# 1Jamie/HMSE

Hardware: AMD Instinct MI355X
Metric: ingest_GiB_per_s (higher is better)
Workload: dtype u8; 1 GPU; full ingest (FastCDC 2/8/32 KiB + SHA-256 dedupe + MinHash-128/LSH 4x32 + dictionary DEFLATE level-9 profile) over 10.00 GB wikipedia; total_bytes=9999220736, seg_size=4194304, collective=none

## Files before the change

### hmse_amd/csrc/l1_deflate.hip

```cpp
#include "common.h"
#include <stdio.h>
#include <stdlib.h>
#include <mutex>

namespace dfl {

constexpr int HB = 12;
constexpr int NBK = 1 << HB;
constexpr uint32_t MINM = 4, MAXM = 258, WMAX = 32768;

__device__ __forceinline__ uint32_t hash4(uint32_t x) { return (x * 0x9E3779B1u) >> (32 - HB); }
__device__ __forceinline__ uint32_t ld32(const uint8_t* p) { uint32_t v; __builtin_memcpy(&v, p, 4); return v; }

__device__ __forceinline__ uint32_t alignb(uint32_t hi, uint32_t lo, uint32_t sh) { return __builtin_amdgcn_alignbyte(hi, lo, sh); }
__device__ __forceinline__ uint32_t ld32a(const uint8_t* W, uint32_t off) {
  const uint32_t* w = (const uint32_t*)(W + (off & ~3u));
  return alignb(w[1], w[0], off);
}
__device__ __forceinline__ void ld64a(const uint8_t* W, uint32_t off, uint32_t& x0, uint32_t& x1) {
  const uint32_t* w = (const uint32_t*)(W + (off & ~3u));
  const uint32_t a = w[0], b = w[1], c = w[2];
  x0 = alignb(b, a, off); x1 = alignb(c, b, off);
}
__device__ __forceinline__ uint32_t sort_key(const uint8_t* W, uint32_t off) {
  const uint32_t* w = (const uint32_t*)(W + (off & ~3u));
  const uint32_t a = w[0], b = w[1];
  return ((alignb(b, a, off) * 0x9E3779B1u) & 0xFFFF0000u) | ((b >> ((off & 3u) * 8u)) & 0x0Fu);
}
template <int N>
__device__ __forceinline__ void ldNa(const uint8_t* W, uint32_t off, uint64_t (&x)[N]) {
  const uint32_t* w = (const uint32_t*)(W + (off & ~3u));
  uint32_t d[2 * N + 1];
#pragma unroll
  for (int u = 0; u < 2 * N + 1; u++) d[u] = w[u];
#pragma unroll
  for (int u = 0; u < N; u++) x[u] = ((uint64_t)alignb(d[2 * u + 2], d[2 * u + 1], off) << 32) | alignb(d[2 * u + 1], d[2 * u], off);
}

__device__ __forceinline__ uint32_t cur_get(const uint32_t* c, uint32_t h) { return (c[h >> 1] >> ((h & 1u) * 16u)) & 0xFFFFu; }
__device__ __forceinline__ uint32_t cur_inc(uint32_t* c, uint32_t h) {
  const uint32_t sh = (h & 1u) * 16u;
  return (atomicAdd(&c[h >> 1], 1u << sh) >> sh) & 0xFFFFu;
}

__device__ __forceinline__ void len_sym(uint32_t len, uint32_t& code, uint32_t& eb, uint32_t& ev) {
  if (len == 258) { code = 285; eb = 0; ev = 0; return; }
  const uint32_t l = len - 3;
  if (l < 8) { code = 257 + l; eb = 0; ev = 0; return; }
  const uint32_t e = (31 - __builtin_clz(l)) - 2;
  code = 257 + 4 * e + 4 + ((l >> e) & 3); eb = e; ev = l & ((1u << e) - 1);
}
__device__ __forceinline__ void dist_sym(uint32_t dist, uint32_t& code, uint32_t& eb, uint32_t& ev) {
  const uint32_t d = dist - 1;
  if (d < 4) { code = d; eb = 0; ev = 0; return; }
  const uint32_t hb = 31 - __builtin_clz(d), e = hb - 1;
  code = 2 * hb + ((d >> e) & 1); eb = e; ev = d & ((1u << e) - 1);
}
__device__ __forceinline__ uint32_t len_extra_bits(uint32_t code) {
  if (code < 265 || code == 285) return 0;
  return (code - 261) >> 2;
}
__device__ __forceinline__ uint32_t dist_extra_bits(uint32_t code) { return code < 4 ? 0 : (code >> 1) - 1; }
__device__ __forceinline__ uint32_t fixed_len(uint32_t s) { return s < 144 ? 8 : s < 256 ? 9 : s < 280 ? 7 : 8; }

__device__ __forceinline__ uint32_t uni32(uint32_t v) { return (uint32_t)__builtin_amdgcn_readfirstlane((int)v); }
__device__ __forceinline__ uint64_t uni64(uint64_t v) { return ((uint64_t)uni32((uint32_t)(v >> 32)) << 32) | uni32((uint32_t)v); }

__device__ __forceinline__ void wave_sync() {
  __builtin_amdgcn_fence(__ATOMIC_ACQ_REL, "wavefront");
  __builtin_amdgcn_wave_barrier();
}

template <int N>
struct HuffScratchT {
  uint32_t key[N];
  uint32_t sorted[N];
  uint32_t w[2 * N];
  uint16_t parent[2 * N];
  uint32_t cnt[32];
};
using HuffL = HuffScratchT<288>;
using HuffD = HuffScratchT<32>;

template <int NT, bool WQ>
struct Small {
  uint32_t lf[288], df[32];
  uint32_t red[NT / 64 + 1];
  uint32_t qhead;
  uint32_t ocnt[4];
  struct { uint32_t ji, job, L, Dl; uint64_t c, cstart, rec_at, dstart; } nx;
  uint32_t pexit[NT / 64], pexit2[NT / 64], pconv[NT / 64];
  uint8_t wtab[WQ ? NT : 64];
};

constexpr int align16(int v) { return (v + 15) & ~15; }

#ifndef HMSE_TCAP_S
#define HMSE_TCAP_S 10048
#define HMSE_TCAP_S2 13952
#define HMSE_TCAP_SG 17408
#define HMSE_TCAP_SG2 22976
#endif
constexpr int NT_S = 1024, TCAP_S = HMSE_TCAP_S, TCAP_S2 = HMSE_TCAP_S2, TCAP_SG = HMSE_TCAP_SG, TCAP_SG2 = HMSE_TCAP_SG2;
constexpr int NT_M = 1024, TCAP_SG3 = 32768;
#ifndef HMSE_NT_B
#define HMSE_NT_B 1024
#endif
constexpr int NT_B = HMSE_NT_B, TCAP_B = 65536, LCAP_B = 32768;

template <int NT, int TCAP, int LCAP_, bool LDSM, bool MDG = false, bool MLG = false, bool NOK = false>
struct Layout {
  static constexpr int LCAP = LCAP_;
  static constexpr int W_OFF = 0;
  static constexpr int W_SZ = align16(TCAP + 64);
  static constexpr int CUR_OFF = W_OFF + W_SZ;
  static constexpr int CUR_SZ = NBK * 2;
  static constexpr int MARK_OFF = CUR_OFF + CUR_SZ;
  static constexpr int MARK_SZ = align16(LCAP / 8 + 16);
  static constexpr int SMALL_OFF = MARK_OFF + MARK_SZ;
  static constexpr int SMALL_SZ = align16((int)sizeof(Small<NT, !LDSM>));
  static constexpr int A_OFF = SMALL_OFF + SMALL_SZ;
  static constexpr int A_SZ = LDSM ? align16(2 * TCAP + 80) : align16(LCAP + 80);
  static constexpr int MD_OFF = A_OFF + A_SZ;
  static constexpr int MD_SZ = (LDSM && !MDG) ? align16(2 * LCAP) : 0;
  static constexpr int ML_OFF = MD_OFF + MD_SZ;
  static constexpr int ML_SZ = (LDSM && !MLG) ? align16(LCAP) : 0;
  static constexpr int K_OFF = ML_OFF + ML_SZ;
  static constexpr int K_SZ = (LDSM && !NOK) ? align16(TCAP + 16) : 0;
  static constexpr int TOTAL = K_OFF + K_SZ;
  static_assert(TOTAL <= 160 * 1024, "one workgroup's LDS image must fit the CU's 160 KiB");
  static_assert(!(LDSM && TCAP <= TCAP_SG2) || TOTAL <= 80 * 1024, "classes S .. SG2 run two workgroups per CU");
  static_assert(sizeof(HuffL) + sizeof(HuffD) <= CUR_SZ, "Huffman scratch must fit the cursor table");
};

template <typename HS>
__device__ void huff_lengths_wave(const uint32_t* freq, uint32_t n, uint32_t limit, uint8_t* lens, HS* hs) {
  const uint32_t lane = lane_id();
  uint32_t used = 0;
  for (uint32_t b = 0; b < n; b += 64) {
    const uint32_t s = b + lane;
    used += (uint32_t)__builtin_popcountll(__ballot(s < n && freq[s] != 0));
  }
  uint32_t dummy0 = 0xFFFFFFFFu, dummy1 = 0xFFFFFFFFu;
  if (used == 0) { dummy0 = 0; dummy1 = 1; }
  else if (used == 1) dummy0 = freq[0] != 0 ? 1u : 0u;
  uint32_t m = 0;
  for (uint32_t b = 0; b < n; b += 64) {
    const uint32_t s = b + lane;
    uint32_t f = s < n ? freq[s] : 0u;
    if (s == dummy0 || s == dummy1) f = 1;
    if (s < n) lens[s] = 0;
    const bool u = f != 0;
    const uint64_t mask = __ballot(u);
    if (u) hs->key[m + (uint32_t)__builtin_popcountll(mask & lanemask_lt())] = (f << 9) | s;
    m += (uint32_t)__builtin_popcountll(mask);
  }
  wave_sync();
  for (uint32_t j = lane; j < m; j += 64) {
    const uint32_t kj = hs->key[j];
    uint32_t r = 0;
    for (uint32_t i = 0; i < m; i++) r += hs->key[i] < kj;
    hs->sorted[r] = kj;
// ... 286 lines not shown
        if (t < a0 - Dl) W[Dl + t] = csrc[t];
        if (t < T - a1) W[a1 + t] = csrc[a1 - Dl + t];
      } else if (t < L) W[Dl + t] = csrc[t];
    }
    if (t < 64) W[T + t] = 0;
    for (uint32_t i = t; i < NBK / 2; i += NT) cur[i] = 0;
    for (uint32_t i = t; i < 288; i += NT) sm.lf[i] = 0;
    if (t < 32) sm.df[t] = 0;
    if (t == 0) sm.qhead = 0;
    if (t < 4) sm.ocnt[t] = 0;
    for (uint32_t i = t * 16; i < L; i += NT * 16) *(uint4*)(mlen + i) = make_uint4(0, 0, 0, 0);
    __syncthreads();

    STAMP(0);
    PF_STAGE(0);
    const uint32_t nh = T >= 4 ? T - 3 : 0;
    for (uint32_t q4 = t * 4u; q4 < nh; q4 += NT * 4u) {
      const uint32_t d0 = *(const uint32_t*)(W + q4), d1 = *(const uint32_t*)(W + q4 + 4u);
      cur_inc(cur, hash4(d0));
      if (q4 + 1u < nh) cur_inc(cur, hash4(alignb(d1, d0, 1u)));
      if (q4 + 2u < nh) cur_inc(cur, hash4(alignb(d1, d0, 2u)));
      if (q4 + 3u < nh) cur_inc(cur, hash4(alignb(d1, d0, 3u)));
    }
    __syncthreads();
    {
      constexpr int PERW = NBK / 2 / NT > 0 ? NBK / 2 / NT : 1;
      uint32_t wv[PERW], sum = 0;
#pragma unroll
      for (int i = 0; i < PERW; i++) {
        const uint32_t idx = t * PERW + i;
        wv[i] = idx < NBK / 2 ? cur[idx] : 0u;
        sum += (wv[i] & 0xFFFFu) + (wv[i] >> 16);
      }
      uint32_t total;
      uint32_t ex = block_exclusive_scan<NT>(sum, sm.red, &total);
#pragma unroll
      for (int i = 0; i < PERW; i++) {
        const uint32_t idx = t * PERW + i;
        const uint32_t lo16 = ex; ex += wv[i] & 0xFFFFu;
        const uint32_t hi16 = ex; ex += wv[i] >> 16;
        if (idx < NBK / 2) cur[idx] = lo16 | (hi16 << 16);
      }
    }
    __syncthreads();
    STAMP(1);
    PF_STAGE(1);
    {
      uint32_t q = t, h = 0, before = 0, hx = 0;
      bool act = q < nh;
      if (act) { hx = sort_key(W, q); h = hx >> (32 - HB); before = cur_get(cur, h); }
      __syncthreads();
      for (uint32_t q0 = 0; q0 < nh; q0 += NT) {
        if (act) S[cur_inc(cur, h)] = (uint16_t)q;
        __syncthreads();
        uint32_t r = 0;
        if (act) {
          const uint32_t after = cur_get(cur, h);
          for (uint32_t jj = before; jj < after; jj++) r += S[jj] < q;
        }
        const uint32_t qn = q0 + NT + t;
        const bool actn = qn < nh;
        uint32_t hn = 0, beforen = 0, hxn = 0;
        if (actn) { hxn = sort_key(W, qn); hn = hxn >> (32 - HB); beforen = cur_get(cur, hn); }
        __syncthreads();
        if (act) { S[before + r] = (uint16_t)q; if constexpr (!NOK) K[before + r] = (uint8_t)((hx & 0x0Fu) | ((hx >> 12) & 0xF0u)); }
        q = qn; act = actn; h = hn; before = beforen; hx = hxn;
      }
      __syncthreads();
    }
    STAMP(2);
    PF_STAGE(2);
    uint32_t* const anch = mark;
    if constexpr (DICT) {
      const uint32_t n_anch = (L + 63u) >> 6;
      for (uint32_t a0 = wave; a0 < n_anch; a0 += NT / 64) {
        const uint32_t pa = Dl + (a0 << 6);
        uint32_t word = 0;
        if (pa + 4 <= T) {
          const uint32_t h = hash4(ld32a(W, pa));
          const uint32_t lo = h ? cur_get(cur, h - 1) : 0u, hi = cur_get(cur, h);
          uint32_t l = lo, r = hi;
          while (l < r) { const uint32_t m = (l + r) >> 1; if ((uint32_t)S[m] < Dl) l = m + 1; else r = m; }
          const uint32_t first = l > lo + 64u ? l - 64u : lo;
          const uint32_t idx = first + lane;
          uint32_t ml = 0, q = 0;
          if (idx < l) {
            q = S[idx];
            if (TCAP <= (int)WMAX || pa - q <= WMAX) {
              uint64_t qa[4], pb[4];
              ldNa<4>(W, q, qa); ldNa<4>(W, pa, pb);
              ml = 32;
#pragma unroll
              for (int u = 3; u >= 0; u--) { const uint64_t x = qa[u] ^ pb[u]; if (x) ml = 8u * u + ((uint32_t)__builtin_ctzll(x) >> 3); }
            }
          }
          uint32_t key = (ml << 8) | lane;
          key = wave_max(key);
          if ((key >> 8) >= 32u) {
            const uint32_t d = pa - (uint32_t)__builtin_amdgcn_readlane((int)q, (int)(key & 63u));
            const uint32_t off = 8u * lane;
            uint32_t n = 8;
            if (pa + off < T) {
              uint64_t xa[1], xb[1];
              ldNa<1>(W, pa + off - d, xa); ldNa<1>(W, pa + off, xb);
              const uint64_t x = xa[0] ^ xb[0];
              if (x) n = (uint32_t)__builtin_ctzll(x) >> 3;
            } else n = 0;
            const uint64_t mm = __ballot(n < 8u);
            uint32_t run = 512;
            if (mm) { const uint32_t fl = (uint32_t)__builtin_ctzll(mm); run = 8u * fl + (uint32_t)__builtin_amdgcn_readlane((int)n, (int)fl); }
            if (run > T - pa) run = T - pa;
            word = d | (run << 16);
          }
        }
        anch[a0] = word;
      }
      __syncthreads();
    }
    auto hint_of = [&](uint32_t p, uint32_t maxlen, uint32_t& bq) -> uint32_t {
      const uint32_t a0 = (p - Dl) >> 6;
      uint32_t bm = 0; bq = 0;
#pragma unroll
      for (uint32_t back = 0; back < 2; back++) {
        if (a0 < back) continue;
        const uint32_t w = anch[a0 - back];
        const uint32_t d = w & 0xFFFFu, run = w >> 16, pa = Dl + ((a0 - back) << 6);
        if (w == 0 || p < pa || d > p || p - d >= Dl) continue;
        uint32_t m = 0;
        if (run >= 512u) m = maxlen;
        else if (pa + run > p) m = (pa + run - p) < maxlen ? (pa + run - p) : maxlen;
        if (m > bm) { bm = m; bq = p - d; }
      }
      return bm;
    };
    if constexpr (DICT) {
      for (uint32_t x = t; x < L; x += NT) {
        const uint32_t p = Dl + x;
        if (p + 4 > T) continue;
        const uint32_t maxlen = (T - p) < MAXM ? (T - p) : MAXM;
        uint32_t bq;
        const uint32_t bm = hint_of(p, maxlen, bq);
        if (bm >= 16u) { mlen[x] = (uint8_t)(bm - 3); mdist[x] = (uint16_t)(p - bq); }
      }
    }
#if defined(HMSE_NO_ORD)
    constexpr bool ORD = false;
#elif defined(HMSE_NO_DICT_ORD)
    constexpr bool ORD = !DICT && LDSM;
#else
    constexpr bool ORD = LDSM;
#endif
    uint32_t* const ord = (uint32_t*)(a.scratch2 + (size_t)blockIdx.x * a.scratch2_stride + 98304u);
    if constexpr (ORD) {
      constexpr int ITER = (TCAP + NT - 1) / NT;
      const uint32_t wv = uni32(wave);
      uint32_t pk[(ITER + 2) / 3];
#pragma unroll
      for (int w = 0; w < (ITER + 2) / 3; w++) pk[w] = 0;
      uint32_t n0 = 0, n1 = 0, n2 = 0, n3 = 0;
      {
        const uint32_t last = nh ? nh - 1u : 0u;
        constexpr int G = DICT ? 2 : ITER > 12 ? 4 : 8;
#pragma unroll
        for (int g = 0; g < ITER; g += G) {
          uint32_t pv[G], hv[G], lv[G];
#pragma unroll
          for (int u = 0; u < G; u++) if (g + u < ITER) { const uint32_t r = (wv << 6) + (uint32_t)(g + u) * NT + lane; pv[u] = S[r < last ? r : last]; }
#pragma unroll
          for (int u = 0; u < G; u++) if (g + u < ITER) hv[u] = ld32a(W, pv[u]) * 0x9E3779B1u;
#pragma unroll
          for (int u = 0; u < G; u++) if (g + u < ITER) lv[u] = cur_get(cur, ((hv[u] >> (32 - HB)) - 1u) & (uint32_t)(NBK - 1));
#pragma unroll
          for (int u = 0; u < G; u++) if (g + u < ITER) {
            const int it = g + u;
            const uint32_t r = (wv << 6) + (uint32_t)it * NT + lane;
            uint32_t km = r - ((hv[u] >> (32 - HB)) ? lv[u] : 0u);
            km = km < a.depth ? km : a.depth;
            km = km < 63u ? km : 63u;
            km = r < nh ? km : 0u;
            if constexpr (DICT) {
              const uint32_t pp = pv[u];
              uint32_t bq;
              const uint32_t bm = pp >= Dl ? hint_of(pp, (T - pp) < MAXM ? (T - pp) : MAXM, bq) : 16u;
              km = bm >= 16u ? 0u : km;
            }
            pk[it / 3] |= (km | ((hv[u] >> 10) & 0x3C0u)) << (10 * (it % 3));
            n0 += (uint32_t)__builtin_popcountll(__ballot(km >= 24u)); n1 += (uint32_t)__builtin_popcountll(__ballot(km >= 12u && km < 24u));
            n2 += (uint32_t)__builtin_popcountll(__ballot(km >= 4u && km < 12u)); n3 += (uint32_t)__builtin_popcountll(__ballot(km >= 1u && km < 4u));
          }
        }
      }
      uint32_t bv = 0;
      if (lane < 4u) bv = atomicAdd(&sm.ocnt[lane], lane == 0u ? n0 : lane == 1u ? n1 : lane == 2u ? n2 : n3);
      uint32_t b0 = (uint32_t)__builtin_amdgcn_readlane((int)bv, 0), b1 = (uint32_t)__builtin_amdgcn_readlane((int)bv, 1),
               b2 = (uint32_t)__builtin_amdgcn_readlane((int)bv, 2), b3 = (uint32_t)__builtin_amdgcn_readlane((int)bv, 3);
      __syncthreads();
      {
        const uint32_t c0 = uni32(sm.ocnt[0]), c1 = uni32(sm.ocnt[1]), c2 = uni32(sm.ocnt[2]);
        b1 += c0; b2 += c0 + c1; b3 += c0 + c1 + c2;
      }
#pragma unroll
      for (int it = 0; it < ITER; it++) {
        const uint32_t r0 = (wv << 6) + (uint32_t)it * NT;
        if (r0 < nh) {
          const uint32_t kv = (pk[it / 3] >> (10 * (it % 3))) & 0x3FFu, km = kv & 63u;
          const uint64_t m0 = __ballot(km >= 24u), m1 = __ballot(km >= 12u && km < 24u), m2 = __ballot(km >= 4u && km < 12u), m3 = __ballot(km >= 1u && km < 4u);
          if (km != 0u) {
            const uint64_t mm = km >= 24u ? m0 : km >= 12u ? m1 : km >= 4u ? m2 : m3;
            const uint32_t pos = (km >= 24u ? b0 : km >= 12u ? b1 : km >= 4u ? b2 : b3) + mbcnt64(mm);
            ord[pos] = (r0 + lane) | (kv << 15);
          }
          b0 += (uint32_t)__builtin_popcountll(m0); b1 += (uint32_t)__builtin_popcountll(m1);
          b2 += (uint32_t)__builtin_popcountll(m2); b3 += (uint32_t)__builtin_popcountll(m3);
        }
      }
      __syncthreads();
      STAMP(8);
    }
    STAMP(6);
    PF_STAGE(3);
    {
      enum { FETCH = 0, PROBE = 1, EXTEND = 2, DONE = 3 };
#ifndef HMSE_FETCH_BATCH
#define HMSE_FETCH_BATCH 16
#endif
#ifndef HMSE_FETCH_BATCH_DICT
#define HMSE_FETCH_BATCH_DICT 8
#endif
      constexpr uint32_t FETCH_BATCH = DICT ? HMSE_FETCH_BATCH_DICT : HMSE_FETCH_BATCH;
      uint32_t st = FETCH, i = 0, p = 0, kk = 0, kmax = 0, best = 0, bd = 0, probe = 0, maxlen = 0, ml = 0, q = 0, qn = 0, kn = 0;
      uint32_t pw0 = 0, pw1 = 0;
#ifndef HMSE_NO_PROBE16
      uint32_t pw2 = 0, pw3 = 0;
#endif
      uint32_t pkey = 0;
      auto rejects = [&](uint32_t kb) -> bool {
        if constexpr (NOK) return best >= 4 && kb != (pw1 & 0xFFu);
        else { const uint32_t x = kb ^ pkey; return (x & 0xF0u) != 0 || (best >= 4 && (x & 0x0Fu) != 0); }
      };
      uint64_t wq_mask = 0; uint32_t wq_base = 0; bool wq_done = false;
      const uint32_t nh_s = uni32(nh);
      const uint32_t n_ord = ORD ? uni32(sm.ocnt[0]) + uni32(sm.ocnt[1]) + uni32(sm.ocnt[2]) + uni32(sm.ocnt[3]) : nh_s;
      uint8_t* const wtab = sm.wtab + (wave << 6);
      auto begin_walk = [&](uint32_t ii, uint32_t pp) {
        i = ii; p = pp;
        qn = i ? S[i - 1] : 0u;
        kn = NOK ? (uint32_t)W[qn + 4] : (i ? (uint32_t)K[i - 1] : 0u);
#ifndef HMSE_NO_PROBE16
        { uint64_t pp__[2]; ldNa<2>(W, p, pp__); pw0 = (uint32_t)pp__[0]; pw1 = (uint32_t)(pp__[0] >> 32); pw2 = (uint32_t)pp__[1]; pw3 = (uint32_t)(pp__[1] >> 32); }
#else
        ld64a(W, p, pw0, pw1);
#endif
        const uint32_t hxp = pw0 * 0x9E3779B1u;
        const uint32_t h = hxp >> (32 - HB);
        pkey = (pw1 & 0x0Fu) | ((hxp >> 12) & 0xF0u);
        const uint32_t lo = h ? cur_get(cur, h - 1) : 0u;
        maxlen = (T - p) < MAXM ? (T - p) : MAXM;
        kmax = i - lo;
        if (kmax > a.depth) kmax = a.depth;
        best = MINM - 1; bd = 0; probe = pw0; kk = 1;
#ifdef HMSE_DFL_STAMPS
        if (DICT && t == 0) stamp_acc[7]++;
#endif
        if (kmax != 0) st = PROBE;
      };
      auto begin_walk_listed = [&](uint32_t e) {
        i = e & 0x7FFFu; kmax = (e >> 15) & 63u;
        p = S[i];
        qn = S[i - 1];
        kn = NOK ? (uint32_t)W[qn + 4] : (uint32_t)K[i - 1];
#ifndef HMSE_NO_PROBE16
        { uint64_t pp__[2]; ldNa<2>(W, p, pp__); pw0 = (uint32_t)pp__[0]; pw1 = (uint32_t)(pp__[0] >> 32); pw2 = (uint32_t)pp__[1]; pw3 = (uint32_t)(pp__[1] >> 32); }
#else
        ld64a(W, p, pw0, pw1);
#endif
        pkey = (pw1 & 0x0Fu) | ((e >> 17) & 0xF0u);
        if (kmax == 63u) {
          const uint32_t h = hash4(pw0), lo = h ? cur_get(cur, h - 1) : 0u;
          kmax = i - lo < a.depth ? i - lo : a.depth;
        }
        maxlen = (T - p) < MAXM ? (T - p) : MAXM;
        best = MINM - 1; bd = 0; probe = pw0; kk = 1;
#ifdef HMSE_DFL_STAMPS
        if (DICT && t == 0) stamp_acc[7]++;
#endif
        st = PROBE;
      };
      const uint32_t trip_budget = (nh + 64u) * (a.depth + 16u);
      uint32_t trips = 0;
      for (;;) {
#ifdef HMSE_DFL_STAMPS
        if (t == 0) stamp_acc[13]++;
#endif
        if (++trips > uni32(trip_budget)) {
#ifdef HMSE_DIAG
          const uint64_t sf = __ballot(st == FETCH), sp = __ballot(st == PROBE), se = __ballot(st == EXTEND);
          if (lane == 0) printf("[dfl] trip budget: job %u k %llu L %u Dl %u nh %u wave %u qhead %u wq_base %u wq_mask %llx wq_done %d FETCH %llx PROBE %llx EXTEND %llx p %u kk %u kmax %u best %u ml %u maxlen %u q %u\n",
                                ji, (unsigned long long)k, L, Dl, nh, wave, sm.qhead, wq_base, (unsigned long long)wq_mask, (int)wq_done, (unsigned long long)sf, (unsigned long long)sp, (unsigned long long)se, p, kk, kmax, best, ml, maxlen, q);
#endif
          if (lane == 0) atomicOr(a.status, 16u);
          break;
        }
        uint64_t need = uni64(__ballot(st == FETCH));
        if constexpr (DICT && !ORD) {
          for (int it = 0; need != 0 && it < 6; it++) {
            if (wq_mask == 0) {
              if (wq_done) break;
              uint32_t b = 0;
              if (lane == 0) b = atomicAdd(&sm.qhead, 64u);
              b = uni32(b);
              if (b >= nh_s) { wq_done = true; break; }
              wq_base = b;
              const uint32_t ii = b + lane;
              bool work = false;
              if (ii < nh_s) {
                const uint32_t pp = S[ii];
                if (pp >= Dl) {
                  const uint32_t mx = (T - pp) < MAXM ? (T - pp) : MAXM;
                  uint32_t bq;
                  const uint32_t bm = hint_of(pp, mx, bq);
                  work = bm < 16u;
                }
              }
              wq_mask = uni64(__ballot(work));
              if (wq_mask == 0) continue;
            }
            const uint32_t navail = (uint32_t)__builtin_popcountll(wq_mask), nneed = (uint32_t)__builtin_popcountll(need);
            const uint32_t take_n = navail < nneed ? navail : nneed;
            const bool has = (wq_mask >> lane) & 1ull;
            const uint32_t rm = mbcnt64(wq_mask);
            if (has && rm < take_n) wtab[rm] = (uint8_t)lane;
            wave_sync();
            const bool isneed = (need >> lane) & 1ull;
            const uint32_t rn = mbcnt64(need);
            uint32_t got = 0xFFFFFFFFu;
            if (isneed && rn < take_n) got = wq_base + (uint32_t)wtab[rn];
            wave_sync();
            wq_mask &= ~uni64(__ballot(has && rm < take_n));
            need &= ~uni64(__ballot(isneed && rn < take_n));
            if (got != 0xFFFFFFFFu) begin_walk(got, (uint32_t)S[got]);
          }
          if (wq_done && wq_mask == 0 && st == FETCH) st = DONE;
        } else if (need && ((uint32_t)__builtin_popcountll(need) >= FETCH_BATCH || uni64(__ballot(st == PROBE || st == EXTEND)) == 0)) {
          const uint32_t leader = (uint32_t)__builtin_ctzll(need);
          uint32_t base = 0;
          if (lane == leader) base = atomicAdd(&sm.qhead, (uint32_t)__builtin_popcountll(need));
          base = (uint32_t)__builtin_amdgcn_readlane((int)base, (int)leader);
          if (st == FETCH) {
            const uint32_t f = base + mbcnt64(need);
            if (f >= n_ord) st = DONE;
            else if constexpr (ORD) begin_walk_listed(ord[f]);
            else begin_walk(f, (uint32_t)S[f]);
          }
        }
        if (uni64(__ballot(st != DONE)) == 0) break;
#ifdef HMSE_DFL_STAMPS
        const uint64_t occP__ = __ballot(st == PROBE), occE__ = __ballot(st == EXTEND);
        if (t == 0) {
          const uint32_t nP = (uint32_t)__builtin_popcountll(occP__), nE = (uint32_t)__builtin_popcountll(occE__);
          const uint32_t nF = (uint32_t)__builtin_popcountll(need);
          stamp_acc[16] += nF != 0; stamp_acc[17] += nF; stamp_acc[18] += nP != 0; stamp_acc[19] += nP; stamp_acc[20] += nE != 0; stamp_acc[21] += nE;
        }
#endif
        bool fin = false;
#ifdef HMSE_EXT_MIN
        const uint64_t em__ = uni64(__ballot(st == EXTEND));
        const bool run_ext = (uint32_t)__builtin_popcountll(em__) >= (uint32_t)HMSE_EXT_MIN || uni64(__ballot(st == PROBE)) == 0;
#else
        constexpr bool run_ext = true;
#endif
        if (st == PROBE) {
          q = qn;
          uint32_t kb = kn;
          if (kk < kmax) { qn = S[i - kk - 1]; kn = NOK ? (uint32_t)W[qn + 4] : (uint32_t)K[i - kk - 1]; }
          if (!NOK && rejects(kb) && kk < kmax && !(TCAP > (int)WMAX && p - q > WMAX) ) {
            kk++;
            q = qn; kb = kn;
            if (kk < kmax) { qn = S[i - kk - 1]; kn = NOK ? (uint32_t)W[qn + 4] : (uint32_t)K[i - kk - 1]; }
          }
          fin = true; ml = 0;
          if (TCAP > (int)WMAX && p - q > WMAX) kk = kmax;
          else if (rejects(kb)) { }
          else {
            const uint32_t cprobe = ld32a(W, q + best - 3);
            uint32_t c0, c1;
            ld64a(W, q, c0, c1);
            uint32_t x;
            if (cprobe != probe) { }
            else if ((x = c0 ^ pw0) != 0) ml = (uint32_t)__builtin_ctz(x) >> 3;
            else if ((x = c1 ^ pw1) != 0) ml = 4 + ((uint32_t)__builtin_ctz(x) >> 3);
#ifndef HMSE_NO_PROBE16
            else if (maxlen > 8) {
              uint32_t c2, c3;
              ld64a(W, q + 8, c2, c3);
              if ((x = c2 ^ pw2) != 0) ml = 8 + ((uint32_t)__builtin_ctz(x) >> 3);
              else if ((x = c3 ^ pw3) != 0) ml = 12 + ((uint32_t)__builtin_ctz(x) >> 3);
              else { ml = 16; if (maxlen > 16) { fin = false; st = EXTEND; } }
            } else ml = 8;
#else
            else { ml = 8; if (maxlen > 8) { fin = false; st = EXTEND; } }
#endif
          }
        } else if (st == EXTEND && run_ext) {
          if constexpr (!LDSM || TCAP > TCAP_SG2) {
            uint64_t da[8], db[8];
            ldNa<8>(W, q + ml, da); ldNa<8>(W, p + ml, db);
            uint32_t adv = 64;
            bool hit = false;
#pragma unroll
            for (int u = 7; u >= 0; u--) { const uint64_t x = da[u] ^ db[u]; if (x) { adv = 8 * u + ((uint32_t)__builtin_ctzll(x) >> 3); hit = true; } }
            ml += adv;
            if (hit || ml >= maxlen) fin = true;
          } else {
            uint64_t qa[4], pa[4];
            ldNa<4>(W, q + ml, qa); ldNa<4>(W, p + ml, pa);
            const uint64_t x = qa[0] ^ pa[0], y = qa[1] ^ pa[1], z = qa[2] ^ pa[2], w = qa[3] ^ pa[3];
            if (x) { ml += (uint32_t)__builtin_ctzll(x) >> 3; fin = true; }
            else if (y) { ml += 8 + ((uint32_t)__builtin_ctzll(y) >> 3); fin = true; }
            else if (z) { ml += 16 + ((uint32_t)__builtin_ctzll(z) >> 3); fin = true; }
            else if (w) { ml += 24 + ((uint32_t)__builtin_ctzll(w) >> 3); fin = true; }
            else { ml += 32; if (ml >= maxlen) fin = true; }
          }
        }
        if (fin) {
          if (ml > maxlen) ml = maxlen;
          bool pos_done = false;
          if (ml > best) {
            best = ml; bd = p - q;
            if (ml == maxlen) pos_done = true; else probe = ld32a(W, p + best - 3);
          }
          if (++kk > kmax) pos_done = true;
          st = PROBE;
          if (pos_done) {
            if (best >= MINM) { mlen[p - Dl] = (uint8_t)(best - 3); mdist[p - Dl] = (uint16_t)bd; }
            st = FETCH;
          }
        }
      }
    }
    __syncthreads();
    for (uint32_t i = t; i < (L >> 5) + 2; i += NT) mark[i] = 0;
    STAMP(3);
    PF_STAGE(4);
    const uint8_t* mlen_c = mlen;
    {
      uint8_t* stage = nullptr;
      if constexpr (!LDSM) stage = smem + LY::A_OFF;
      else if constexpr (MLG) {
        const uint32_t joff = (2u * (L + 1u) + 15u) & ~15u;
        if (joff + L + 16u <= (uint32_t)LY::A_SZ) stage = smem + LY::A_OFF + joff;
      }
      if (stage) {
        __syncthreads();
        for (uint32_t i = t * 16; i < L; i += NT * 16) { const uint4 v = *(const uint4*)(mlen_c + i); *(uint4*)(stage + i) = v; }
        mlen_c = stage;
        __syncthreads();
      }
    }
    const uint16_t* const mdist_c = mdist;
    uint8_t* const rec_c = rec;
    auto take = [&](uint32_t x) -> bool {
      const uint32_t ml = mlen_c[x];
      return ml != 0 && !(x + 1 < L && mlen_c[x + 1] > ml);
    };
    for (uint32_t x = t; x <= L; x += NT) {
      uint32_t nx = L;
      if (x < L) { nx = x + (take(x) ? (uint32_t)mlen_c[x] + 3u : 1u); if (nx > L) nx = L; }
      jump[x] = (uint16_t)nx;
    }
    __syncthreads();
    STAMP(11);
    PF_STAGE(5);
    {
      constexpr uint32_t NW = NT / 64;
      const uint32_t SEG = (((L + NW - 1) / NW) + 63u) & ~63u;
      {
        const uint32_t sw = wave * SEG;
        const uint32_t send = (sw + SEG) < L ? (sw + SEG) : L;
        uint32_t curp = sw;
#ifndef HMSE_DFL_PW
#define HMSE_DFL_PW 1
#endif
        constexpr int PWX = HMSE_DFL_PW;
        const uint32_t sw_s = uni32(sw), send_s = uni32(send);
        for (uint32_t wb0 = sw_s; wb0 < send_s; wb0 += 64u * PWX) {
          uint32_t hop[PWX], rlo[PWX], rhi[PWX], wendv[PWX];
#pragma unroll
          for (int u = 0; u < PWX; u++) {
            const uint32_t wb = wb0 + 64u * u;
            const uint32_t x = wb + lane;
            hop[u] = (wb < send_s && x < L) ? (uint32_t)jump[x] : L;
            wendv[u] = (wb + 64) < send_s ? (wb + 64) : send_s;
            rlo[u] = lane < 32 ? 1u << lane : 0u; rhi[u] = lane >= 32 ? 1u << (lane - 32) : 0u;
          }
#pragma nounroll
          for (int r = 0; r < 6; r++) {
            bool inside[PWX], any = false;
#pragma unroll
            for (int u = 0; u < PWX; u++) { inside[u] = (wb0 + 64u * u) < send_s && hop[u] < wendv[u]; any = any || inside[u]; }
            if (__ballot(any) == 0) break;
            uint32_t h2[PWX], l2[PWX], g2[PWX];
#pragma unroll
            for (int u = 0; u < PWX; u++) {
              const int src = (int)(inside[u] ? hop[u] - (wb0 + 64u * u) : lane);
              h2[u] = (uint32_t)__shfl((int)hop[u], src, 64);
              l2[u] = (uint32_t)__shfl((int)rlo[u], src, 64); g2[u] = (uint32_t)__shfl((int)rhi[u], src, 64);
            }
#pragma unroll
            for (int u = 0; u < PWX; u++) {
              rlo[u] |= inside[u] ? l2[u] : 0u;
              rhi[u] |= inside[u] ? g2[u] : 0u;
              hop[u] = inside[u] ? h2[u] : hop[u];
            }
          }
#pragma unroll
          for (int u = 0; u < PWX; u++) {
            const uint32_t wb = wb0 + 64u * u;
            if (wb < send_s) {
              uint64_t m = 0;
              if (curp < wendv[u]) {
                const int el = (int)(curp - wb);
                m = ((uint64_t)(uint32_t)__builtin_amdgcn_readlane((int)rhi[u], el) << 32) | (uint32_t)__builtin_amdgcn_readlane((int)rlo[u], el);
                curp = (uint32_t)__builtin_amdgcn_readlane((int)hop[u], el);
              }
              mark[wb >> 5] = (uint32_t)m; mark[(wb >> 5) + 1] = (uint32_t)(m >> 32);
            }
          }
        }
        sm.pexit[wave] = curp;
      }
      __syncthreads();
      STAMP(12);
      auto stitch = [&](uint32_t w, uint32_t e, uint32_t chain_exit, bool intact, bool& conv_out) -> uint32_t {
        const uint32_t sw = w * SEG;
        const uint32_t send = (sw + SEG) < L ? (sw + SEG) : L;
        conv_out = true;
        if (intact && e == sw) return chain_exit;
        for (uint32_t wb = sw; wb < send && (wb + 64 <= e || e >= send); wb += 64)
          { mark[wb >> 5] = 0; mark[(wb >> 5) + 1] = 0; }
        uint32_t curp = e;
        bool conv = false;
        for (uint32_t wb = e & ~63u; wb < send && !conv; wb += 64) {
          const uint32_t x = wb + lane;
          const uint32_t nv = x < L ? (uint32_t)jump[x] : L;
          const uint64_t spec = (uint64_t)mark[wb >> 5] | ((uint64_t)mark[(wb >> 5) + 1] << 32);
          const uint32_t wend = (wb + 64) < send ? (wb + 64) : send;
          uint64_t m = 0;
          while (curp < wend) {
            if ((spec >> (curp - wb)) & 1ull) { conv = true; break; }
            m |= 1ull << (curp - wb);
            curp = (uint32_t)__builtin_amdgcn_readlane((int)nv, (int)(curp - wb));
          }
          if (conv) m |= spec & ~((1ull << (curp - wb)) - 1ull);
          mark[wb >> 5] = (uint32_t)m; mark[(wb >> 5) + 1] = (uint32_t)(m >> 32);
        }
        conv_out = conv;
        return conv ? chain_exit : curp;
      };
      {
        const uint32_t sw = wave * SEG;
        bool conv = true;
        uint32_t ex = sm.pexit[wave];
        if (wave > 0 && sw < L) ex = stitch(wave, sm.pexit[wave - 1], sm.pexit[wave], true, conv);
        wave_sync();
        sm.pexit2[wave] = ex; sm.pconv[wave] = (wave == 0 || sw >= L || conv) ? 1u : 0u;
      }
      __syncthreads();
      if (wave == 0) {
        uint32_t first_bad = NW;
        for (uint32_t w = 0; w < NW; w++) if (sm.pconv[w] == 0u) { first_bad = w; break; }
        if (first_bad < NW) {
          uint32_t tru = sm.pexit2[first_bad];
          for (uint32_t w = first_bad + 1; w < NW; w++) {
            if (w * SEG >= L) break;
            bool cv;
            tru = stitch(w, tru, sm.pexit2[w], false, cv);
          }
        }
      }
    }
    __syncthreads();
    STAMP(4);
    PF_STAGE(6);
    {
      uint32_t* const tok = (uint32_t*)(rec_c + rec_tok_off());
      const uint32_t ppt = (L + NT - 1) / NT;
      const uint32_t p0 = t * ppt < L ? t * ppt : L, p1 = (p0 + ppt) < L ? (p0 + ppt) : L;
// ... 728 lines not shown
```

Before: 31.43 GiB/s.

## Resolve nearest hash-chain candidates via cross-lane DPP compare before walk

The sorted-position ordering pass now overlaps wave rows by UG lanes. Each lane compares its 16-byte prefix against the UG preceding sorted positions using DPP lane shifts and ffbl, which gives an early best match for the nearest chain candidates. Positions that are fully resolved this way skip the per-position walk. Partially resolved ones start the walk at candidate UG+1 with a seeded best length, and 255 marks a match of 16 bytes or more that needs a full restart. This cuts probe/extend iterations in the serial walk loop, at the cost of extra ALU and register work and more subtle correctness conditions such as the bd!=0 guard.

```diff
diff --git a/hmse_amd/csrc/l1_deflate.hip b/hmse_amd/csrc/l1_deflate.hip
--- a/hmse_amd/csrc/l1_deflate.hip
+++ b/hmse_amd/csrc/l1_deflate.hip
@@ -8,6 +8,14 @@
 constexpr int HB = 12;
 constexpr int NBK = 1 << HB;
 constexpr uint32_t MINM = 4, MAXM = 258, WMAX = 32768;
+
+#ifndef HMSE_UNIFORM_G
+#define HMSE_UNIFORM_G 3
+#endif
+constexpr int UG = HMSE_UNIFORM_G;
+static_assert(UG >= 0 && UG <= 16, "HMSE_UNIFORM_G: 0 .. 16 levels");
+__device__ __forceinline__ uint32_t ffbl(uint32_t v) { uint32_t r; asm("v_ffbl_b32 %0, %1" : "=v"(r) : "v"(v)); return r; }
+__device__ __forceinline__ uint32_t lane_below(uint32_t v) { return (uint32_t)__builtin_amdgcn_update_dpp(0, (int)v, 0x138, 0xf, 0xf, true); }
 
 __device__ __forceinline__ uint32_t hash4(uint32_t x) { return (x * 0x9E3779B1u) >> (32 - HB); }
 __device__ __forceinline__ uint32_t ld32(const uint8_t* p) { uint32_t v; __builtin_memcpy(&v, p, 4); return v; }
@@ -600,7 +608,8 @@
 #endif
     uint32_t* const ord = (uint32_t*)(a.scratch2 + (size_t)blockIdx.x * a.scratch2_stride + 98304u);
     if constexpr (ORD) {
-      constexpr int ITER = (TCAP + NT - 1) / NT;
+      constexpr int NWV = NT / 64, RW = 64 - UG;
+      constexpr int ITER = (TCAP + NWV * RW - 1) / (NWV * RW);
       const uint32_t wv = uni32(wave);
       uint32_t pk[(ITER + 2) / 3];
 #pragma unroll
@@ -608,29 +617,76 @@
       uint32_t n0 = 0, n1 = 0, n2 = 0, n3 = 0;
       {
         const uint32_t last = nh ? nh - 1u : 0u;
-        constexpr int G = DICT ? 2 : ITER > 12 ? 4 : 8;
+#ifndef HMSE_UNIFORM_STAGE
+#define HMSE_UNIFORM_STAGE 2
+#endif
+        constexpr int G = UG > 0 ? (DICT ? 1 : HMSE_UNIFORM_STAGE) : DICT ? 2 : ITER > 12 ? 4 : 8;
 #pragma unroll
         for (int g = 0; g < ITER; g += G) {
+          if constexpr (UG > 0) __builtin_amdgcn_sched_barrier(0);
           uint32_t pv[G], hv[G], lv[G];
-#pragma unroll
-          for (int u = 0; u < G; u++) if (g + u < ITER) { const uint32_t r = (wv << 6) + (uint32_t)(g + u) * NT + lane; pv[u] = S[r < last ? r : last]; }
-#pragma unroll
-          for (int u = 0; u < G; u++) if (g + u < ITER) hv[u] = ld32a(W, pv[u]) * 0x9E3779B1u;
+          uint32_t pw[UG > 0 ? G : 1][4];
+#pragma unroll
+          for (int u = 0; u < G; u++) if (g + u < ITER) {
+            uint32_t r = ((uint32_t)(g + u) * NWV + wv) * RW + lane;
+            if constexpr (UG > 0) r = r < (uint32_t)UG ? 0u : r - (uint32_t)UG;
+            pv[u] = S[r < last ? r : last];
+          }
+#pragma unroll
+          for (int u = 0; u < G; u++) if (g + u < ITER) {
+            if constexpr (UG > 0) {
+              uint64_t pp__[2];
+              ldNa<2>(W, pv[u], pp__);
+              pw[u][0] = (uint32_t)pp__[0]; pw[u][1] = (uint32_t)(pp__[0] >> 32); pw[u][2] = (uint32_t)pp__[1]; pw[u][3] = (uint32_t)(pp__[1] >> 32);
+              hv[u] = pw[u][0] * 0x9E3779B1u;
+            } else hv[u] = ld32a(W, pv[u]) * 0x9E3779B1u;
+          }
 #pragma unroll
           for (int u = 0; u < G; u++) if (g + u < ITER) lv[u] = cur_get(cur, ((hv[u] >> (32 - HB)) - 1u) & (uint32_t)(NBK - 1));
 #pragma unroll
           for (int u = 0; u < G; u++) if (g + u < ITER) {
             const int it = g + u;
-            const uint32_t r = (wv << 6) + (uint32_t)it * NT + lane;
+            const uint32_t r = ((uint32_t)it * NWV + wv) * RW + lane - (uint32_t)UG;
             uint32_t km = r - ((hv[u] >> (32 - HB)) ? lv[u] : 0u);
             km = km < a.depth ? km : a.depth;
             km = km < 63u ? km : 63u;
-            km = r < nh ? km : 0u;
+            km = (r < nh && lane >= (uint32_t)UG) ? km : 0u;
             if constexpr (DICT) {
               const uint32_t pp = pv[u];
               uint32_t bq;
               const uint32_t bm = pp >= Dl ? hint_of(pp, (T - pp) < MAXM ? (T - pp) : MAXM, bq) : 16u;
               km = bm >= 16u ? 0u : km;
+            }
+            if constexpr (UG > 0) {
+              const uint32_t pp = pv[u];
+              const uint32_t mx = (T - pp) < MAXM ? (T - pp) : MAXM;
+              uint32_t c0 = pw[u][0], c1 = pw[u][1], c2 = pw[u][2], c3 = pw[u][3], cq = pp;
+              uint32_t bkey = ((MINM - 1) << 16) | 0xFFFFu;
+              const uint32_t mx16 = mx < 16u ? mx : 16u;
+#pragma unroll
+              for (uint32_t lv_k = 1; lv_k <= (uint32_t)UG; lv_k++) {
+                c0 = lane_below(c0); c1 = lane_below(c1); c2 = lane_below(c2); c3 = lane_below(c3); cq = lane_below(cq);
+                const uint32_t f0 = ffbl(c0 ^ pw[u][0]), f1 = ffbl(c1 ^ pw[u][1]) | 32u, f2 = ffbl(c2 ^ pw[u][2]) | 64u, f3 = ffbl(c3 ^ pw[u][3]) | 96u;
+                uint32_t fb = f0 < f1 ? f0 : f1; fb = fb < f2 ? fb : f2; fb = fb < f3 ? fb : f3;
+                uint32_t m = fb >> 3;
+                const uint32_t cap = lv_k <= km ? mx16 : 0u;
+                m = m < cap ? m : cap;
+                const uint32_t key = (m << 16) | cq;
+                bkey = key > bkey ? key : bkey;
+              }
+              const uint32_t bst = bkey >> 16, bdd = pp - (bkey & 0xFFFFu);
+              const bool scratch = bst == 16u && mx > 16u, open = bst != mx;
+#ifdef HMSE_DFL_STAMPS
+              { const uint64_t f__ = __ballot(km != 0u && !scratch && (!open || km <= (uint32_t)UG)), s__ = __ballot(km != 0u && scratch);
+                if (t == 0) { stamp_acc[22] += (uint32_t)__builtin_popcountll(f__); stamp_acc[23] += (uint32_t)__builtin_popcountll(s__); } }
+#endif
+              if (km != 0u) {
+                if (scratch) mlen[pp - Dl] = 255u;
+                else {
+                  if (bst >= MINM) { mlen[pp - Dl] = (uint8_t)(bst - 3); mdist[pp - Dl] = (uint16_t)bdd; }
+                  if (!open || km <= (uint32_t)UG) km = 0u;
+                }
+              }
             }
             pk[it / 3] |= (km | ((hv[u] >> 10) & 0x3C0u)) << (10 * (it % 3));
             n0 += (uint32_t)__builtin_popcountll(__ballot(km >= 24u)); n1 += (uint32_t)__builtin_popcountll(__ballot(km >= 12u && km < 24u));
@@ -647,16 +703,18 @@
         const uint32_t c0 = uni32(sm.ocnt[0]), c1 = uni32(sm.ocnt[1]), c2 = uni32(sm.ocnt[2]);
         b1 += c0; b2 += c0 + c1; b3 += c0 + c1 + c2;
       }
+      uint32_t lane2 = lane;
+      if constexpr (UG > 0) asm volatile("" : "+v"(lane2));
 #pragma unroll
       for (int it = 0; it < ITER; it++) {
-        const uint32_t r0 = (wv << 6) + (uint32_t)it * NT;
-        if (r0 < nh) {
+        const uint32_t r0 = ((uint32_t)it * NWV + wv) * RW - (uint32_t)UG;
+        if (r0 + (uint32_t)UG < nh) {
           const uint32_t kv = (pk[it / 3] >> (10 * (it % 3))) & 0x3FFu, km = kv & 63u;
           const uint64_t m0 = __ballot(km >= 24u), m1 = __ballot(km >= 12u && km < 24u), m2 = __ballot(km >= 4u && km < 12u), m3 = __ballot(km >= 1u && km < 4u);
           if (km != 0u) {
             const uint64_t mm = km >= 24u ? m0 : km >= 12u ? m1 : km >= 4u ? m2 : m3;
             const uint32_t pos = (km >= 24u ? b0 : km >= 12u ? b1 : km >= 4u ? b2 : b3) + mbcnt64(mm);
-            ord[pos] = (r0 + lane) | (kv << 15);
+            ord[pos] = (r0 + lane2) | (kv << 15);
           }
           b0 += (uint32_t)__builtin_popcountll(m0); b1 += (uint32_t)__builtin_popcountll(m1);
           b2 += (uint32_t)__builtin_popcountll(m2); b3 += (uint32_t)__builtin_popcountll(m3);
@@ -729,6 +787,15 @@
         }
         maxlen = (T - p) < MAXM ? (T - p) : MAXM;
         best = MINM - 1; bd = 0; probe = pw0; kk = 1;
+        if constexpr (UG > 0) {
+          const uint32_t m = mlen[p - Dl];
+          if (m != 255u) {
+            best = m + 3u; kk = (uint32_t)UG + 1u;
+            qn = S[i - kk];
+            kn = NOK ? (uint32_t)W[qn + 4] : (uint32_t)K[i - kk];
+            probe = ld32a(W, p + best - 3);
+          }
+        }
 #ifdef HMSE_DFL_STAMPS
         if (DICT && t == 0) stamp_acc[7]++;
 #endif
@@ -880,7 +947,7 @@
           if (++kk > kmax) pos_done = true;
           st = PROBE;
           if (pos_done) {
-            if (best >= MINM) { mlen[p - Dl] = (uint8_t)(best - 3); mdist[p - Dl] = (uint16_t)bd; }
+            if (best >= MINM && (UG == 0 || !ORD || bd != 0)) { mlen[p - Dl] = (uint8_t)(best - 3); mdist[p - Dl] = (uint16_t)bd; }
             st = FETCH;
           }
         }
```

Result: slower. 30.75 GiB/s (-2.2%).
